# wcaarls/grl

Measured on AMD Instinct MI355X. Metric: env-steps/sec (batched rollouts), pendulum SARSA-tc, higher is better.
Workload: dtype f64

## Files before the change

### grl_amd/csrc/grlx_env_server.h

```cpp
#pragma once

namespace grlx {

struct __attribute__((aligned(16))) MailUnit { double v; unsigned long long seq; };
constexpr int kCandUnits = 5;
constexpr int kCandSlots = 4;
struct __attribute__((aligned(1024))) EnvMail {
  unsigned long long cmd[4];
  MailUnit reset[3];
  unsigned long long pad0[6];
  unsigned long long stats[16];
  union {
    MailUnit by_unit[2][kCandUnits][kCandSlots];
    MailUnit by_cand[2][3][kCandUnits];
  } cand;
  unsigned long long pad1[16];
};
static_assert(sizeof(EnvMail) == kEnvMailBytes, "one mailbox = kEnvMailBytes");
static_assert(offsetof(EnvMail, stats) + 15 * sizeof(unsigned long long) == kEnvMailFlagOffset, "the flag grlx_env_server_counts reads");
static_assert(offsetof(EnvMail, stats) + 14 * sizeof(unsigned long long) == kEnvMailUniformOffset, "the count grlx_uniform_pass_counts reads");

typedef __attribute__((address_space(1))) unsigned long long env_gu64;
typedef unsigned int mail_u32x4 __attribute__((ext_vector_type(4)));
#define GRLX_RLX_AGENT __ATOMIC_RELAXED, __HIP_MEMORY_SCOPE_AGENT
constexpr unsigned kMailReset = 3u, kMailExit = 4u;
constexpr unsigned kFetchPolls = 400u;
constexpr unsigned kFirstFetchPolls = 8000u;
constexpr unsigned kServerStartPolls = 20000u;
constexpr unsigned kServerIdlePolls = 400000u;

__device__ __forceinline__ void mail_store(void *p, unsigned long long v) { __hip_atomic_store((env_gu64 *)p, v, GRLX_RLX_AGENT); }
__device__ __forceinline__ unsigned long long mail_load(const void *p) { return __hip_atomic_load((env_gu64 *)p, GRLX_RLX_AGENT); }
__device__ __forceinline__ void mail_setprio(unsigned p)
{
  if (p == 1) __builtin_amdgcn_s_setprio(1);
  else if (p == 2) __builtin_amdgcn_s_setprio(2);
  else if (p == 3) __builtin_amdgcn_s_setprio(3);
}
__device__ __forceinline__ unsigned long long mail_clock()
{
  unsigned long long t;
  asm volatile("s_memtime %0\n\ts_waitcnt lgkmcnt(0)" : "=s"(t)::"memory");
  return t;
}

__device__ __forceinline__ void unit_store(MailUnit *p, double v, unsigned long long seq)
{
  const unsigned long long b = (unsigned long long)__double_as_longlong(v);
  mail_u32x4 d;
  d.x = (unsigned)b; d.y = (unsigned)(b >> 32); d.z = (unsigned)seq; d.w = (unsigned)(seq >> 32);
  asm volatile("global_store_dwordx4 %0, %1, off sc1\n\ts_nop 1" ::"v"(p), "v"(d) : "memory");
}
template <int I, int STRIDE = 1>
__device__ __forceinline__ void unit_store_at(MailUnit *p, double v, unsigned long long seq)
{
  const unsigned long long b = (unsigned long long)__double_as_longlong(v);
  mail_u32x4 d;
  d.x = (unsigned)b; d.y = (unsigned)(b >> 32); d.z = (unsigned)seq; d.w = (unsigned)(seq >> 32);
  asm volatile("global_store_dwordx4 %0, %1, off offset:%2 sc1\n\ts_nop 1" ::"v"(p), "v"(d), "n"(I * STRIDE * (int)sizeof(MailUnit)) : "memory");
}
template <int N>
__device__ __forceinline__ bool units_load(const MailUnit *p, unsigned long long seq, double *v)
{
  static_assert(N == 3, "");
  mail_u32x4 d[N];
  asm volatile("global_load_dwordx4 %0, %3, off sc1\n\t"
               "global_load_dwordx4 %1, %3, off offset:16 sc1\n\t"
               "global_load_dwordx4 %2, %3, off offset:32 sc1\n\t"
               "s_waitcnt vmcnt(0)"
               : "=&v"(d[0]), "=&v"(d[1]), "=&v"(d[2])
               : "v"(p)
               : "memory");
  bool ok = true;
#pragma unroll
  for (int i = 0; i < N; ++i)
  {
    ok = ok && (((unsigned long long)d[i].w << 32) | d[i].z) == seq;
    v[i] = __longlong_as_double((long long)(((unsigned long long)d[i].y << 32) | d[i].x));
  }
  return ok;
}

struct MailRef {
  EnvMail *all;
  uint32_t r;
  __device__ __forceinline__ EnvMail *get() const { return all + in_reg(r); }
  __device__ __forceinline__ EnvMail *operator->() const { return get(); }
};
__device__ __forceinline__ void mail_send(EnvMail *m, unsigned long long seq, unsigned op) { mail_store(&m->cmd[seq & 3u], (seq << 8) | op); }
__device__ __forceinline__ void mail_send_reset(EnvMail *m, unsigned long long seq, const double *x)
{
  static_assert(offsetof(EnvMail, reset) == 2 * sizeof(MailUnit), "reset[i] is unit 2 + i of the mailbox");
  MailUnit *u = reinterpret_cast<MailUnit *>(m);
  unit_store_at<2>(u, x[0], seq);
  unit_store_at<3>(u, x[1], seq);
  unit_store_at<4>(u, x[2], seq);
  mail_send(m, seq, kMailReset);
}
__device__ __forceinline__ void mail_send(const MailRef &m, unsigned long long seq, unsigned op) { mail_send(m.get(), seq, op); }
__device__ __forceinline__ void mail_send_reset(const MailRef &m, unsigned long long seq, const double *x) { mail_send_reset(m.get(), seq, x); }

template <bool BY_UNIT>
struct MailBox {
  __amdgpu_buffer_rsrc_t rs;
  unsigned at;
};
template <bool BY_UNIT>
__device__ __forceinline__ MailBox<BY_UNIT> mailbox_of(const DevParams &P, int r, int j)
{
  MailBox<BY_UNIT> b;
  b.rs = __builtin_amdgcn_make_buffer_rsrc((void *)P.env_mail, 0, (int)((size_t)P.n_replicas * kEnvMailBytes), 0x00020000);
  b.at = (unsigned)r * (unsigned)kEnvMailBytes + (unsigned)offsetof(EnvMail, cand) + (unsigned)(j < kCandUnits ? j : 0) * (unsigned)((BY_UNIT ? kCandSlots : 1) * sizeof(MailUnit));
  return b;
}
template <bool BY_UNIT>
__device__ __forceinline__ mail_u32x4 mail_prefetch(const MailBox<BY_UNIT> &b, unsigned long long seq, int a)
{
  const unsigned off = BY_UNIT ? b.at + (((unsigned)seq & 1u) * (unsigned)(kCandUnits * kCandSlots) + (unsigned)a) * (unsigned)sizeof(MailUnit)
                               : b.at + (((unsigned)seq & 1u) * 3u + (unsigned)a) * (unsigned)(kCandUnits * sizeof(MailUnit));
  return __builtin_amdgcn_raw_buffer_load_b128(b.rs, off, 0, 16);
}
template <int ENV, bool BY_UNIT>
__device__ __forceinline__ bool mail_take(const DevParams &N, const MailBox<BY_UNIT> &b, mail_u32x4 d, unsigned long long seq, int a, int g,
                                          unsigned long long gmask, double *x, double *obs, double &reward, int &terminal, uint32_t &status,
                                          unsigned long long *polled = nullptr)
{
  static_assert(ENV == GRLX_ENV_PENDULUM, "the pendulum's mailbox");
  bool ok = false;
  unsigned polls = 0;
  for (;;)
  {
    const bool mine = (((unsigned long long)d.w << 32) | d.z) == seq;
    if ((__ballot(mine) & gmask) == gmask) { ok = true; break; }
    if (++polls > (seq <= 1u ? kFirstFetchPolls : kFetchPolls)) break;
    d = mail_prefetch(b, seq, a);
  }
  if (polled) *polled += polls;
  if (!ok) return false;
  const double v = __longlong_as_double((long long)(((unsigned long long)d.y << 32) | d.x));
  const int base = g * 16;
  x[0] = lane_fetch(v, base + 0);
  x[1] = lane_fetch(v, base + 1);
  x[2] = lane_fetch(v, base + 2);
  obs[0] = lane_fetch(v, base + 3);
  obs[1] = x[1];
  reward = lane_fetch(v, base + 4);
  terminal = x[2] > N.timeout ? 1 : 0;
  if (!Env<ENV>::in_domain(x)) status |= ST_DOMAIN;
  return true;
}
template <int ENV, bool BY_UNIT>
__device__ __forceinline__ bool mail_take_wave(const DevParams &N, const MailBox<BY_UNIT> &b, mail_u32x4 d, unsigned long long seq, int a, int g,
                                               double *x, double *obs, double &reward, int &terminal, uint32_t &status,
// ... 24 lines not shown
  return true;
}
__device__ __forceinline__ void mail_nothing_in_flight() { __builtin_amdgcn_s_waitcnt(0x0F70); }
__device__ __forceinline__ mail_u32x4 mail_prefetch_all(const MailBox<true> &b, unsigned long long seq, int j)
{
  const unsigned jj = (j >= kCandUnits && j < 3 * kCandUnits) ? (unsigned)j : 0u;
  const unsigned off = b.at + ((jj % (unsigned)kCandUnits) * (unsigned)kCandSlots + jj / (unsigned)kCandUnits) * (unsigned)sizeof(MailUnit) +
                       ((unsigned)seq & 1u) * (unsigned)(kCandUnits * kCandSlots * sizeof(MailUnit));
  return __builtin_amdgcn_raw_buffer_load_b128(b.rs, off, 0, 16);
}
__device__ __forceinline__ bool mail_vote_all(const MailBox<true> &b, mail_u32x4 &d, unsigned long long seq, int j, unsigned long long *polled = nullptr)
{
  unsigned polls = 0;
  while (!__all((((unsigned long long)d.w << 32) | d.z) == seq))
  {
    if (++polls > kFetchPolls)
    {
      if (polled) *polled += polls;
      return false;
    }
    d = mail_prefetch_all(b, seq, j);
  }
  if (polled) *polled += polls;
  return true;
}
template <int ENV>
__device__ __forceinline__ void mail_hand_round(const DevParams &N, const mail_u32x4 &d, int a, int g, double *x, double *obs, double &reward,
                                                int &terminal, uint32_t &status)
{
  static_assert(ENV == GRLX_ENV_PENDULUM, "the pendulum's mailbox");
  const double v = __longlong_as_double((long long)(((unsigned long long)d.y << 32) | d.x));
  const int base = g * 16 + kCandUnits * a;
  x[0] = lane_fetch(v, base + 0);
  x[1] = lane_fetch(v, base + 1);
  x[2] = lane_fetch(v, base + 2);
  obs[0] = lane_fetch(v, base + 3);
  obs[1] = x[1];
  reward = lane_fetch(v, base + 4);
  terminal = x[2] > N.timeout ? 1 : 0;
  if (!Env<ENV>::in_domain(x)) status |= ST_DOMAIN;
}

template <int ENV, int NA, typename SPEC>
__global__ __launch_bounds__(64) __attribute__((amdgpu_num_vgpr(48))) void env_server_kernel(DevParams P)
{
  static_assert(NA == 3, "sixteen lanes per replica: nine pairs of actions");
  constexpr int S = Env<ENV>::S, D = Env<ENV>::D;
  static_assert(S == 3 && D == 2, "the pendulum's mailbox");
  const DevParams &N = SPEC::numeric(P);
  const int lane = threadIdx.x & 63;
  const int q = lane >> 4, c = lane & 15;
  const int a = c / NA, a2 = c % NA;
  const bool worker = c < NA * NA;
  const int r = blockIdx.x * kReplicasPerWave + q;
  bool done = r >= P.n_replicas || (P.env_tune & 64u) != 0;
  EnvMail *m = P.env_mail + (done ? 0 : r);
  const double act = N.actions[a2];
  unsigned long long expect = 1;
  double cx[S], cobs0 = 0, creward = 0;
#pragma unroll
  for (int i = 0; i < S; ++i) cx[i] = 0;
  unsigned idle = 0;
  bool seen = false;
  mail_setprio((P.env_tune >> 2) & 3u);
  const typename Env<ENV>::ServerConsts ec = Env<ENV>::server_consts();
#ifdef GRLX_ENV_SERVER_STATS
  unsigned long long t_begin = mail_clock(), t_busy = 0, n_cmd = 0, n_idle = 0, n_split = 0, n_batch = 0;
#endif
  const unsigned long long quit_after = (P.env_tune >> 8) & 0xFFFFu;
  const unsigned quit_mask = P.env_tune >> 24;
  const bool leaves = quit_after != 0u && (quit_mask == 0u || ((quit_mask >> q) & 1u) != 0u);
  for (;;)
  {
    if (leaves && expect > quit_after) done = true;
    if (__all(done)) break;
    unsigned long long word = 0;
    bool ready = false;
    if (!done)
    {
      word = mail_load(&m->cmd[expect & 3u]);
      ready = (word >> 8) == expect;
      if ((word >> 8) > expect) done = true;
    }
    if (!__any(ready))
    {
      __builtin_amdgcn_s_sleep(1);
#ifdef GRLX_ENV_SERVER_STATS
      ++n_idle;
#endif
      if (++idle > (seen ? kServerIdlePolls : kServerStartPolls)) break;
      continue;
    }
    seen = true;
    bool progress = false;
#ifdef GRLX_ENV_SERVER_STATS
    const unsigned long long t0 = mail_clock();
    if (!__all(ready || done)) ++n_split;
    ++n_batch;
#endif
    bool step = false;
    unsigned op = 0u;
    if (ready)
    {
      op = (unsigned)(word & 0xFFu);
      if (op == kMailExit)
      {
        done = true;
        progress = true;
      }
      else
        step = true;
    }
    if (rarely(__any(step && op == kMailReset)))
      if (step && op == kMailReset)
      {
        double x[S];
        step = units_load<3>(&m->reset[0], expect, x);
        if (step)
        {
          double obs[D];
          int terminal = 0;
          uint32_t st = 0;
#pragma unroll
          for (int i = 0; i < S; ++i) cx[i] = x[i];
          env_step_consts<ENV>(N, ec, cx, act, obs, creward, terminal, st);
          cobs0 = obs[0];
          op = 0u;
        }
      }
    if (step)
    {
      if (worker && a == (int)op)
      {
        static_assert(NA <= kCandSlots, "slot a2 of every unit is this lane's");
        constexpr bool BY_UNIT = SPEC::kCandByUnit;
        constexpr int STRIDE = BY_UNIT ? kCandSlots : 1;
        MailUnit *u;
        if constexpr (BY_UNIT) u = &m->cand.by_unit[expect & 1u][0][a2];
        else u = &m->cand.by_cand[expect & 1u][a2][0];
        unit_store_at<0, STRIDE>(u, cx[0], expect);
        unit_store_at<1, STRIDE>(u, cx[1], expect);
        unit_store_at<2, STRIDE>(u, cx[2], expect);
        unit_store_at<3, STRIDE>(u, cobs0, expect);
        unit_store_at<4, STRIDE>(u, creward, expect);
      }
      const int src = (lane & ~15) + (int)op * NA + (worker ? a : 0);
      double x[S];
#pragma unroll
      for (int i = 0; i < S; ++i) x[i] = lane_fetch(cx[i], src);
      double obs[D];
      int terminal = 0;
      uint32_t st = 0;
#pragma unroll
      for (int i = 0; i < S; ++i) cx[i] = x[i];
      env_step_consts<ENV>(N, ec, cx, act, obs, creward, terminal, st);
      cobs0 = obs[0];
      ++expect;
      progress = true;
#ifdef GRLX_ENV_SERVER_STATS
      ++n_cmd;
#endif
    }
    if (__any(progress)) idle = 0;
    else if (++idle > kServerIdlePolls) break;
#ifdef GRLX_ENV_SERVER_STATS
    t_busy += mail_clock() - t0;
#endif
  }
#ifdef GRLX_ENV_SERVER_STATS
  if (c == 0 && r < P.n_replicas)
  {
    EnvMail *mm = P.env_mail + r;
    mm->stats[0] = mail_clock() - t_begin;
    mm->stats[1] = t_busy;
    mm->stats[2] = n_cmd;
    mm->stats[3] = n_idle;
    mm->stats[9] = n_split;
    mm->stats[10] = n_batch;
  }
#endif
}

}
```

### grl_amd/csrc/grlx_rollout.h

```cpp
#pragma once

namespace grlx {

__device__ __forceinline__ unsigned long long stamp()
{
  unsigned long long t;
  __builtin_amdgcn_sched_barrier(0);
  asm volatile("s_memtime %0\n\ts_waitcnt lgkmcnt(0)" : "=s"(t)::"memory");
  __builtin_amdgcn_sched_barrier(0);
  return t;
}
#ifdef GRLX_ENV_SERVER_STATS
#define GRLX_STAMPED (DIAG || SERVED)
#else
#define GRLX_STAMPED DIAG
#endif
#define DIAG_STAMP(slot)                                   \
  if (GRLX_STAMPED)                                        \
  {                                                        \
    unsigned long long now__ = stamp();                    \
    diag_sum[slot] += now__ - diag_last;                   \
    diag_last = now__;                                     \
  }

constexpr DevParams make_spec_pendulum_tc()
{
  DevParams P{};
  P.env = GRLX_ENV_PENDULUM;
  P.agent = GRLX_AGENT_SARSA;
  P.trace_kind = GRLX_TRACE_REPLACING;
  P.test_interval = 10;
  P.h = 0.03 / 5;
  P.integration_steps = 5;
  P.timeout = 2.99;
  P.randomization = 0;
  P.A = 3;
  P.actions[0] = -3; P.actions[1] = 0; P.actions[2] = 3;
  P.tile.T = 16; P.tile.D = 3; P.tile.memory = 8388608;
  P.tile.scaling[0] = 16 / 0.31415; P.tile.scaling[1] = 16 / 3.1415; P.tile.scaling[2] = 16 / 3.0;
  P.tile.wrap[0] = 320;
  P.lin.init_min = 0; P.lin.init_range = 1;
  P.lin.out_min = -1.7976931348623157e308; P.lin.out_max = 1.7976931348623157e308;
  P.lin.limit = 1; P.lin.draws_before = 0;
  P.epsilon = 0.05; P.decay_rate = 1; P.decay_min = 0;
  P.alpha = 0.2; P.gamma = 0.97; P.gl = 0.97 * 0.65;
  return P;
}
__device__ const DevParams d_spec_pendulum_tc = make_spec_pendulum_tc();

struct SpecShared {
  static constexpr bool kPerReplica = false;
  static constexpr bool kEarlyTake = false;
  static constexpr bool kCandByUnit = false;
  struct Rep {};
  __device__ static __forceinline__ Rep replica(const SweepParams *, int) { return Rep{}; }
  __device__ static __forceinline__ double alpha(const DevParams &N, const Rep &) { return N.alpha; }
  __device__ static __forceinline__ double gamma(const DevParams &N, const Rep &) { return N.gamma; }
  __device__ static __forceinline__ double gl(const DevParams &N, const Rep &) { return N.gl; }
  __device__ static __forceinline__ double epsilon(const DevParams &N, const Rep &) { return N.epsilon; }
};

template <int AGENT>
struct SpecPendulumTcA : SpecShared {
  static constexpr bool kEarlyTake = true;
  static constexpr bool kCandByUnit = true;
  __device__ static __forceinline__ int agent(const DevParams &) { return AGENT; }
  static bool matches(const DevParams &P)
  {
    constexpr DevParams C = make_spec_pendulum_tc();
    bool ok = P.env == C.env && P.trace_kind == C.trace_kind && P.test_interval == C.test_interval && P.h == C.h &&
              P.integration_steps == C.integration_steps && P.timeout == C.timeout && P.randomization == C.randomization && P.A == C.A &&
              P.tile.T == C.tile.T && P.tile.D == C.tile.D && P.tile.memory == C.tile.memory &&
              P.lin.init_min == C.lin.init_min && P.lin.init_range == C.lin.init_range && P.lin.out_min == C.lin.out_min &&
              P.lin.out_max == C.lin.out_max && P.lin.limit == C.lin.limit && P.lin.draws_before == C.lin.draws_before &&
              P.epsilon == C.epsilon && P.decay_rate == C.decay_rate && P.decay_min == C.decay_min && P.alpha == C.alpha &&
              P.gamma == C.gamma && P.gl == C.gl && P.agent == AGENT;
    for (int i = 0; i < 3; ++i)
      ok = ok && P.actions[i] == C.actions[i] && P.tile.scaling[i] == C.tile.scaling[i] && P.tile.wrap[i] == C.tile.wrap[i];
    return ok;
  }
  __device__ static __forceinline__ const DevParams &numeric(const DevParams &) { return d_spec_pendulum_tc; }
};
using SpecPendulumTc = SpecPendulumTcA<GRLX_AGENT_SARSA>;

inline bool spec_numeric_equal(const DevParams &a, const DevParams &b)
{
  auto tile_eq = [](const TileParams &x, const TileParams &y) {
    bool ok = x.T == y.T && x.D == y.D && x.memory == y.memory;
    for (int i = 0; i < GRLX_MAX_DIMS; ++i) ok = ok && x.scaling[i] == y.scaling[i] && x.wrap[i] == y.wrap[i];
    return ok;
  };
  auto lin_eq = [](const LinearParams &x, const LinearParams &y) {
    return x.init_min == y.init_min && x.init_range == y.init_range && x.out_min == y.out_min && x.out_max == y.out_max &&
           x.limit == y.limit && x.draws_before == y.draws_before;
  };
  bool ok = a.test_interval == b.test_interval && a.env == b.env && a.agent == b.agent && a.trace_kind == b.trace_kind &&
            a.integration_steps == b.integration_steps && a.h == b.h && a.timeout == b.timeout && a.randomization == b.randomization &&
            a.A == b.A && tile_eq(a.tile, b.tile) && lin_eq(a.lin, b.lin) && a.epsilon == b.epsilon && a.decay_rate == b.decay_rate &&
            a.decay_min == b.decay_min && a.alpha == b.alpha && a.gamma == b.gamma && a.gl == b.gl &&
            tile_eq(a.tile_actor, b.tile_actor) && lin_eq(a.lin_actor, b.lin_actor) && a.actor_alpha == b.actor_alpha &&
            a.sigma == b.sigma && a.theta == b.theta && a.ac_decay_rate == b.ac_decay_rate && a.ac_decay_min == b.ac_decay_min &&
            a.ac_step_limit == b.ac_step_limit && a.ac_update_method == b.ac_update_method && a.action_min == b.action_min &&
            a.action_max == b.action_max && a.end_stop_penalty == b.end_stop_penalty && a.action_penalty == b.action_penalty &&
            a.control_step == b.control_step && a.slope_angle == b.slope_angle &&
            a.initial_state_variation == b.initial_state_variation && a.negative_reward == b.negative_reward &&
            a.walker_dt == b.walker_dt && a.kappa == b.kappa && a.beta == b.beta && a.tile_safe == b.tile_safe &&
            a.target_interval == b.target_interval && a.target_tau == b.target_tau;
  for (int i = 0; i < kMaxActions; ++i) ok = ok && a.actions[i] == b.actions[i];
  return ok;
}

constexpr void spec_q_agent_block(DevParams &P)
{
  P.agent = GRLX_AGENT_Q;
  P.trace_kind = GRLX_TRACE_REPLACING;
  P.test_interval = 10;
  P.randomization = 0;
  P.A = 3;
// ... 14 lines not shown
  P.integration_steps = 20;
  P.control_step = 0.2;
  P.h = 0.2 / (double)(size_t)20;
  P.timeout = 100.0;
  P.slope_angle = 0.004; P.initial_state_variation = 0.2; P.negative_reward = -100.0;
  P.walker_dt = 1.0E-6 * (double)(uint64_t)200000 / 20;
  P.action_min = -1.2; P.action_max = 1.2;
  P.actions[0] = -1.2 + (2.4 / 2.) * 0; P.actions[1] = -1.2 + (2.4 / 2.) * 1; P.actions[2] = -1.2 + (2.4 / 2.) * 2;
  P.tile.D = 6;
  P.tile.scaling[0] = 16 / 0.0838; P.tile.scaling[1] = 16 / 0.1047; P.tile.scaling[2] = 16 / 0.1111;
  P.tile.scaling[3] = 16 / 0.2222; P.tile.scaling[4] = 16 / 10.; P.tile.scaling[5] = 16 / 1.2;
  return P;
}
constexpr DevParams make_spec_acrobot_q()
{
  DevParams P{};
  spec_q_agent_block(P);
  P.env = GRLX_ENV_ACROBOT;
  P.integration_steps = 5;
  P.control_step = 0.05;
  P.h = 0.05 / (double)(size_t)5;
  P.timeout = 20.0;
  P.walker_dt = 1.0E-6 * (double)(uint64_t)50000 / 5;
  P.action_min = -1.0; P.action_max = 1.0;
  P.actions[0] = -1.0 + (2.0 / 2.) * 0; P.actions[1] = -1.0 + (2.0 / 2.) * 1; P.actions[2] = -1.0 + (2.0 / 2.) * 2;
  P.tile.D = 5;
  P.tile.scaling[0] = 16 / 0.05; P.tile.scaling[1] = 16 / 0.05; P.tile.scaling[2] = 16 / 0.2; P.tile.scaling[3] = 16 / 0.4;
  P.tile.scaling[4] = 16 / 1.0;
  return P;
}
__device__ const DevParams d_spec_walker_q = make_spec_walker_q();
__device__ const DevParams d_spec_acrobot_q = make_spec_acrobot_q();
struct SpecWalkerQ : SpecShared {
  static constexpr int kEnv = GRLX_ENV_COMPASS_WALKER;
  __device__ static __forceinline__ int agent(const DevParams &) { return GRLX_AGENT_Q; }
  static bool matches(const DevParams &P) { constexpr DevParams C = make_spec_walker_q(); return spec_numeric_equal(P, C); }
  __device__ static __forceinline__ const DevParams &numeric(const DevParams &) { return d_spec_walker_q; }
};
struct SpecAcrobotQ : SpecShared {
  static constexpr int kEnv = GRLX_ENV_ACROBOT;
  __device__ static __forceinline__ int agent(const DevParams &) { return GRLX_AGENT_Q; }
  static bool matches(const DevParams &P) { constexpr DevParams C = make_spec_acrobot_q(); return spec_numeric_equal(P, C); }
  __device__ static __forceinline__ const DevParams &numeric(const DevParams &) { return d_spec_acrobot_q; }
};
struct SpecNone : SpecShared {
  __device__ static __forceinline__ const DevParams &numeric(const DevParams &P) { return P; }
  __device__ static __forceinline__ int agent(const DevParams &P) { return P.agent; }
};
struct SpecSweep {
  __device__ static __forceinline__ const DevParams &numeric(const DevParams &P) { return P; }
  __device__ static __forceinline__ int agent(const DevParams &P) { return P.agent; }
  static constexpr bool kPerReplica = true;
  static constexpr bool kCandByUnit = false;
  struct Rep { double alpha, gamma, gl, epsilon; };
  __device__ static __forceinline__ Rep replica(const SweepParams *sweep, int r)
  {
    const SweepParams &w = sweep[r];
    return Rep{w.alpha, w.gamma, w.gl, w.epsilon};
  }
  __device__ static __forceinline__ double alpha(const DevParams &, const Rep &R) { return R.alpha; }
  __device__ static __forceinline__ double gamma(const DevParams &, const Rep &R) { return R.gamma; }
  __device__ static __forceinline__ double gl(const DevParams &, const Rep &R) { return R.gl; }
  __device__ static __forceinline__ double epsilon(const DevParams &, const Rep &R) { return R.epsilon; }
};

#ifdef GRLX_TWO_WAVES
#define GRLX_ROLLOUT_OCCUPANCY __attribute__((amdgpu_waves_per_eu(2, 2)))
#else
#define GRLX_ROLLOUT_OCCUPANCY
#endif
template <int ENV, int NA, bool DIAG, typename SPEC, bool DEFER, bool ADV, bool TAP, bool SERVED>
__device__ __forceinline__ void rollout_body(const DevParams &P, int n_trials, const SweepParams *sweep = nullptr)
{
  static_assert(!(ADV && DEFER), "the advantage-learning instantiation updates in place");
  constexpr int NROWS = ADV ? 2 * NA : NA + 1;
  const DevParams &N = SPEC::numeric(P);
  constexpr int S = Env<ENV>::S, D = Env<ENV>::D, T = kLanesPerReplica;
  __shared__ double   sh_w[NROWS * 16 * 4];
  __shared__ uint32_t sh_ppos[4 * 16];
  __shared__ double   sh_fb[16 * 4];
  __shared__ uint32_t sh_fbflag[16 * 4];
  __shared__ uint32_t sh_mb[4 * NA * 16];
  __shared__ uint32_t sh_ms[4 * NA * 16];
  __shared__ uint32_t sh_mail[4];
  __shared__ double   sh_res[4 * 16];
  __shared__ uint64_t sh_jump[2048];
  jump_table_to_lds(sh_jump);

  const int lane = threadIdx.x & 63;
  const int g = lane >> 4, j = lane & 15;
  const int r_raw = blockIdx.x * kReplicasPerWave + g;
  const bool live = r_raw < P.n_replicas;
  const int r = live ? r_raw : 0;
  const bool tapped = live && (r == P.tap_replica);
  const unsigned long long gmask = 0xFFFFull << (16 * g);

  ReplicaState &RS = P.states[r];
  double x[S];
#pragma unroll
  for (int i = 0; i < S; ++i) x[i] = RS.x[i];
  uint64_t G = RS.G, TL = RS.TL, S1 = RS.S1;
  double eps_decay = RS.eps_decay;
  int64_t tt = RS.tt, ss = RS.ss;
  uint64_t test_steps = RS.test_steps;
  uint32_t status = RS.status, rows = RS.rows, inserted = 0;

  const typename SPEC::Rep rep = SPEC::replica(sweep, r);
  const Table tab = table_of(P, 0, r);
  ReplicaState RSc;
  RSc.TL0 = RS.TL0;
  RSc.lazy_base[0] = RS.lazy_base[0];
  UpdateParams up;
  up.out_min = N.lin.out_min;
  up.out_max = N.lin.out_max;
  up.limit = N.lin.limit != 0;
  up.ee = SPEC::gl(N, rep);
  up.cut = (N.trace_kind == GRLX_TRACE_REPLACING) ? 0.01 : 0.0001;
  up.use_trace = N.trace_kind == GRLX_TRACE_REPLACING;
  up.dW = up.dT = 0;

  double acts[NA];
#pragma unroll
  for (int a = 0; a < NA; ++a) acts[a] = N.actions[a];
  uint32_t key_act[NA];
#pragma unroll
  for (int a = 0; a < NA; ++a)
    key_act[a] = in_reg(murmur_key(tile_coord<T>(N.tile, D, tile_quant(N.tile, D, N.actions[a]), j)));
  const uint32_t key_j = in_reg(murmur_key(j));

  LaneShare lshare;
  lshare.src[0] = g * 16; lshare.src[1] = g * 16 + 1; lshare.src[2] = g * 16 + 2;
  lshare.role3 = j % 3; lshare.role2 = j & 1;

  constexpr bool EXT = SERVED;
  static_assert(!SERVED || (DEFER && !DIAG && !TAP && !ADV && ENV == GRLX_ENV_PENDULUM && NA == 3), "what the environment server works for");
  MailRef mail = {nullptr, 0u};
  unsigned long long mseq = 0;
  bool srv = false;
  unsigned n_uniform = 0;
#ifdef GRLX_ENV_SERVER_STATS
  unsigned long long st_wait = 0, st_polls = 0, st_fetch = 0, st_begin = mail_clock();
#endif
  MailBox<SPEC::kCandByUnit> mbox;
  mail_u32x4 mpre = {0u, 0u, 0u, 0u};
  if constexpr (EXT)
  {
    srv = live && P.env_mail != nullptr;
    mail = MailRef{P.env_mail, (uint32_t)r};
    mbox = mailbox_of<SPEC::kCandByUnit>(P, r, j);
    mail_setprio(P.env_tune & 3u);
  }

  TraceRegs tr;
  trace_init(tr);
  int tr_len_ref = 0;
  bool pd = false, pd_sh = false;
  double pd_dW = 0, pd_dT = 0, pd_wp = 0;
  uint32_t pd_pos = kInvalidPos;
  unsigned long long diag_sum[8] = {0, 0, 0, 0, 0, 0, 0, 0}, diag_last = 0;
  if (GRLX_STAMPED) diag_last = stamp();

  for (int trial = 0; trial < n_trials; ++trial)
  {
    const bool act = live && !(P.steps_budget != 0u && (uint64_t)ss >= P.steps_budget);
    if (!__any(act)) break;
    const int ti = N.test_interval;
    const int test = (ti >= 0 && tt % (ti + 1) == ti) ? 1 : 0;
    double total_reward = 0, time = 0;
    const int subtrials = (test && P.test_trials > 1) ? P.test_trials : 1;
    for (int st = 0; st < P.test_trials; ++st)
    {
    const bool episode = act && st < subtrials;
    if (!__any(episode)) break;
    double obs[D], reward = 0;
    int terminal = 0;
    bool running = episode;

    if (episode)
    {
      Env<ENV>::start(N, test, TL, G, x);
      Env<ENV>::observe(N, x, obs);
      if constexpr (EXT)
        if (srv)
        {
          ++mseq;
          if (j == 0) mail_send_reset(mail, mseq, x);
        }
    }
    double action = 0;
    int    action_index = 0;
    uint32_t p_pos = kInvalidPos, p_slot = 0;
    bool   p_sh = false;
    double wp_seen = 0;
    uint32_t pos_prev[NA];
#pragma unroll
    for (int a = 0; a < NA; ++a) pos_prev[a] = 0u;
    if (!test) tr_len_ref = 0;
    bool first = true;

    for (;;)
    {
      if constexpr (SERVED)
      {
        static_assert(!Env<ENV>::kAbsorbing, "has_next is taken as true");
        if (__all(live && running && !first && srv && !test && pd) && !(P.env_tune & 16u))
        {
          auto take_classic = [&]() -> bool {
#ifdef GRLX_ENV_SERVER_STATS
            const unsigned long long tf0 = mail_clock();
            const bool stepped = mail_take_wave<ENV>(N, mbox, mpre, mseq - 1, action_index, g, x, obs, reward, terminal, status, &st_polls);
            st_wait += mail_clock() - tf0;
            ++st_fetch;
            return stepped;
#else
            return mail_take_wave<ENV>(N, mbox, mpre, mseq - 1, action_index, g, x, obs, reward, terminal, status);
#endif
          };
          constexpr bool EARLY = SPEC::kEarlyTake;
          bool go = true;
          if constexpr (EARLY)
          {
            DIAG_STAMP(0)
            go = take_classic();
            mail_nothing_in_flight();
          }
          if (go)
          do
          {
            if constexpr (!EARLY)
            {
              DIAG_STAMP(0)
              if (!take_classic()) break;
            }
            ++n_uniform;
            total_reward += reward;
            time += 1;
            DIAG_STAMP(1)

            uint32_t slot[NA];
// ... 117 lines not shown
              }
            }
            auto pass_tail = [&]() {
              DIAG_STAMP(4)
              {
                double target = reward;
                if (SPEC::agent(P) == GRLX_AGENT_SARSA)
                  target += SPEC::gamma(N, rep) * pick<double, NA>(q, a_next);
                else if (SPEC::agent(P) == GRLX_AGENT_EXPECTED_SARSA)
                {
                  const double de = eps_decay * SPEC::epsilon(N, rep);
                  double v = 0;
#pragma unroll
                  for (int kk = 0; kk < NA; ++kk)
                  {
                    double d = (q[kk] == best) ? 1. / man : 0.;
                    if (d == 1) d = 1 - de;
                    d += de / NA;
                    v += q[kk] * d;
                  }
                  target += SPEC::gamma(N, rep) * v;
                }
                else
                {
                  double v = -__builtin_inf();
#pragma unroll
                  for (int kk = 0; kk < NA; ++kk) v = fmax(v, q[kk]);
                  target += SPEC::gamma(N, rep) * v;
                }
                const double delta = target - qsa;
                pd_dW = SPEC::alpha(N, rep) * (target - qsa);
                pd_dT = SPEC::alpha(N, rep) * delta;
                pd_pos = p_pos;
                status |= (p_pos == kInvalidPos) ? ST_BAD_POS : 0u;
                pd_sh = p_sh;
                pd_wp = wp;
              }
              DIAG_STAMP(5)
              ss++;
              action_index = a_next;
              p_pos = pick<uint32_t, NA>(pos, a_next);
              p_sh = pick<bool, NA>(sh, a_next);
              wp_seen = pick<double, NA>(w, a_next);
              if (terminal) running = false;
              if (ev.pos != kInvalidPos) value_store(tab, ev.pos, ev.val);
            };
            if constexpr (EARLY)
            {
              if (!early)
              {
                if (!terminal)
                {
                  ++mseq;
                  if (j == 0) mail_send(mail, mseq, (unsigned)a_next);
                }
                mpre = mail_prefetch(mbox, mseq - 1, a_next);
                DIAG_STAMP(1)
                pass_tail();
                break;
              }
              mail_nothing_in_flight();
              ++mseq;
              if (j == 0) mail_send(mail, mseq, (unsigned)a_next);
              DIAG_STAMP(1)
              pass_tail();
              DIAG_STAMP(0)
              mail_hand_round<ENV>(N, mall, a_next, g, x, obs, reward, terminal, status);
            }
            else
            {
              if (!terminal)
              {
                ++mseq;
                if (j == 0) mail_send(mail, mseq, (unsigned)a_next);
                mpre = mail_prefetch(mbox, mseq - 1, a_next);
              }
              pass_tail();
            }
          } while (EARLY || __all(running));
          action = pick<double, NA>(acts, action_index);
        }
      }
      if (!__any(running || pd)) break;
      uint32_t slot[NA];
      Lookup lk[NA];
      BucketRegs br[NA];
      double wp = 0;
      double wprev[NA];
#pragma unroll
      for (int a = 0; a < NA; ++a) wprev[a] = 0;
      bool has_next = false, update = false;
      if (running)
      {
        DIAG_STAMP(0)
        if (!first)
        {
          bool stepped = false;
          if constexpr (EXT)
            if (srv)
            {
#ifdef GRLX_ENV_SERVER_STATS
              const unsigned long long tf0 = mail_clock();
              stepped = mail_take<ENV>(N, mbox, mpre, mseq - 1, action_index, g, gmask, x, obs, reward, terminal, status, &st_polls);
              st_wait += mail_clock() - tf0;
              ++st_fetch;
#else
              stepped = mail_take<ENV>(N, mbox, mpre, mseq - 1, action_index, g, gmask, x, obs, reward, terminal, status);
#endif
              if (!stepped)
              {
                srv = false;
                ++mseq;
                if (j == 0) mail_send(mail, mseq, kMailExit);
              }
            }
          if (!stepped)
            env_step<ENV, true, LaneShare>(N, x, action, obs, reward, terminal, status, lshare);
          total_reward += reward;
          time += 1;
        }
        has_next = first || !Env<ENV>::kAbsorbing || terminal != 2;
        update = !first && !test;
        DIAG_STAMP(1)

        if (has_next)
        {
          uint32_t hpre = 449u ^ (uint32_t)(D + 2);
#pragma unroll
          for (int i = 0; i < D; ++i)
            hpre = murmur_mix(hpre, tile_coord<T>(N.tile, i, tile_quant(N.tile, i, obs[i]), j));
          const uint32_t hpm = hpre * 0x5bd1e995u;
#pragma unroll
          for (int a = 0; a < NA; ++a)
          {
            uint32_t h = hpm ^ key_act[a];
            h = murmur_absorb(h, key_j);
            const uint32_t hm = murmur_final(h), mem = (uint32_t)N.tile.memory;
            slot[a] = ((mem & (mem - 1u)) == 0u) ? (hm & (mem - 1u)) : (hm % mem);
          }
        }
        DIAG_STAMP(2)
        __builtin_amdgcn_fence(__ATOMIC_SEQ_CST, "workgroup");
        DIAG_STAMP(6)
        if (update) wp = DEFER ? wp_seen : value_load(tab, p_pos);
        if (ADV && update)
        {
#pragma unroll
          for (int a = 0; a < NA; ++a) wprev[a] = value_load(tab, pos_prev[a]);
        }
        if (has_next) table_issue<NA>(tab, slot, lk, br);
      }

      Evicted ev;
      ev.n = 0u; ev.pos = kInvalidPos; ev.val = 0;
      if (DEFER)
      {
        DIAG_STAMP(7)
        if (pd)
        {
          sh_ppos[g * 16 + j] = pd_pos;
          sh_fbflag[j * 4 + g] = 0u;
        }
        wave_sync();
        if (pd)
        {
          up.dW = pd_dW;
// ... 91 lines not shown
          sum /= 16;
          sh_res[g * 16 + j] = sum;
        }
        wave_sync();
        if (has_next)
        {
#pragma unroll
          for (int a = 0; a < NA; ++a) q[a] = clampd(sh_res[g * 16 + a], up.out_min, up.out_max);
        }
        double qsa = 0;
        double qprev[NA];
#pragma unroll
        for (int a = 0; a < NA; ++a) qprev[a] = 0;
        if (update)
        {
          if (ADV)
          {
#pragma unroll
            for (int a = 0; a < NA; ++a) qprev[a] = clampd(sh_res[g * 16 + NA + a], up.out_min, up.out_max);
            qsa = pick<double, NA>(qprev, action_index);
          }
          else
            qsa = clampd(sh_res[g * 16 + NA], up.out_min, up.out_max);
        }

        int a_next = 0;
        int mai = 0, man = 1;
        double best = 0;
        if (has_next)
        {
          findmax<NA>(q, mai, man, best);
          if (test)
          {
            a_next = (man > 1) ? tie_break<NA>(q, best, man, G) : mai;
          }
          else
          {
            if (time == 0.) eps_decay = fmax(eps_decay * N.decay_rate, N.decay_min);
            S1 = lcg_next(S1);
            double rnd = lcg_double(S1);
            if (rnd < eps_decay * SPEC::epsilon(N, rep))
            {
              G = lcg_next(G);
              a_next = (int)(lcg_long(G) % (uint32_t)NA);
            }
            else
              a_next = (man > 1) ? tie_break<NA>(q, best, man, G) : mai;
          }
        }
        if constexpr (EXT)
          if (srv && running && has_next && !(!first && terminal))
          {
            ++mseq;
            if (j == 0) mail_send(mail, mseq, (unsigned)a_next);
            if (!(P.env_tune & 16u))
              mpre = mail_prefetch(mbox, mseq - 1, a_next);
          }

        DIAG_STAMP(4)
        double delta = 0;
        if (update)
        {
          double target = reward;
          if (ADV)
          {
            double v = -__builtin_inf();
#pragma unroll
            for (int kk = 0; kk < NA; ++kk) v = fmax(v, qprev[kk]);
            target = v + (reward - v) / N.kappa;
            if (has_next)
            {
              v = -__builtin_inf();
#pragma unroll
              for (int kk = 0; kk < NA; ++kk) v = fmax(v, q[kk]);
              target += N.gamma * v / N.kappa;
            }
          }
          else if (has_next)
          {
            if (SPEC::agent(P) == GRLX_AGENT_SARSA)
              target += SPEC::gamma(N, rep) * pick<double, NA>(q, a_next);
            else if (SPEC::agent(P) == GRLX_AGENT_EXPECTED_SARSA)
            {
              const double de = eps_decay * SPEC::epsilon(N, rep);
              double v = 0;
#pragma unroll
              for (int kk = 0; kk < NA; ++kk)
              {
                double d = (q[kk] == best) ? 1. / man : 0.;
                if (d == 1) d = 1 - de;
                d += de / NA;
                v += q[kk] * d;
              }
              target += SPEC::gamma(N, rep) * v;
            }
            else
            {
              double v = -__builtin_inf();
#pragma unroll
              for (int kk = 0; kk < NA; ++kk) v = fmax(v, q[kk]);
              target += SPEC::gamma(N, rep) * v;
            }
          }
          delta = target - qsa;
          const double dW = SPEC::alpha(N, rep) * (target - qsa);
          const double dT = SPEC::alpha(N, rep) * delta;
          if (DEFER)
// ... 77 lines not shown
        if (!first && terminal) running = false;
        first = false;
      }
      if (DEFER && ev.pos != kInvalidPos) value_store(tab, ev.pos, ev.val);
    }

    if (!test) trace_flush(tr, tab, true);
    }

    if (act && (ti >= 0 ? test : 1))
    {
      if (rows < (uint32_t)P.max_rows)
      {
        if (j == 0)
        {
          size_t at = (size_t)rows * (size_t)P.n_replicas + (size_t)r;
          P.row_reward[at] = total_reward / (double)subtrials;
          P.row_time[at] = time / (double)subtrials;
          P.row_steps[at] = ss;
          P.row_trial[at] = (ti >= 0) ? (tt + 1 - (tt + 1) / (ti + 1)) : tt;
        }
        rows++;
      }
      else
        status |= ST_ROWS_FULL;
    }
    tt += act ? 1 : 0;
  }

  if (DIAG && P.diag_out && lane == 0)
    for (int k = 0; k < 8; ++k) P.diag_out[(size_t)blockIdx.x * 8 + k] = diag_sum[k];

  if constexpr (EXT)
  {
#ifdef GRLX_ENV_SERVER_STATS
    if (live && j == 0 && P.env_mail)
    {
      mail->stats[4] = mail_clock() - st_begin;
      mail->stats[5] = st_wait;
      mail->stats[6] = st_fetch;
      mail->stats[7] = st_polls;
      mail->stats[8] = srv ? 1 : 0;
      for (int k = 0; k < 8; ++k) mail->pad1[k] = diag_sum[k];
    }
#endif
    if (live && j == 0 && P.env_mail)
    {
      mail->stats[14] = n_uniform;
      mail->stats[15] = srv ? 1u : 2u;
    }
    if (srv)
    {
      ++mseq;
      if (j == 0) mail_send(mail, mseq, kMailExit);
    }
  }

  uint32_t ins = inserted;
#pragma unroll
  for (int off = 8; off > 0; off >>= 1) ins += __shfl_xor(ins, off, 16);
  if (live && j == 0)
  {
#pragma unroll
    for (int i = 0; i < S; ++i) RS.x[i] = x[i];
    RS.G = G;
    RS.TL = TL;
    RS.S1 = S1;
    RS.eps_decay = eps_decay;
    RS.tt = tt;
    RS.ss = ss;
    RS.test_steps = test_steps;
    RS.n_slots[0] += ins;
    RS.rows = rows;
  }
  uint32_t st = status;
#pragma unroll
  for (int off = 8; off > 0; off >>= 1) st |= __shfl_xor(st, off, 16);
  if (live && j == 0) RS.status = st;
}

template <int ENV, int NA, bool DIAG, typename SPEC, bool DEFER = !DIAG, bool ADV = false, bool TAP = !DEFER>
__global__ __launch_bounds__(64) GRLX_ROLLOUT_OCCUPANCY void rollout_kernel(DevParams P, int n_trials)
{
  rollout_body<ENV, NA, DIAG, SPEC, DEFER, ADV, TAP, false>(P, n_trials);
}

template <int ENV, int NA>
__global__ __launch_bounds__(64) GRLX_ROLLOUT_OCCUPANCY void rollout_sweep_kernel(DevParams P, int n_trials, const SweepParams *sweep)
{
  rollout_body<ENV, NA, false, SpecSweep, true, false, false, false>(P, n_trials, sweep);
}

template <int NA, typename SPEC>
__global__ __launch_bounds__(64) __attribute__((amdgpu_num_vgpr(208))) void rollout_served_kernel(DevParams P, int n_trials)
{
  rollout_body<GRLX_ENV_PENDULUM, NA, false, SPEC, true, false, false, true>(P, n_trials);
}


}
```

### grl_amd/runner.py

```python
import collections
import ctypes as C
import math

import numpy as np

from . import capi


def pendulum_sarsa_config(n_replicas=1, **overrides) -> capi.Config:
    lib = capi.load()
    cfg = capi.Config()
    lib.grlx_config_pendulum_sarsa(C.byref(cfg))
    cfg.n_replicas = n_replicas
    for k, v in overrides.items():
        setattr(cfg, k, v)
    return cfg


def cart_pole_ac_config(n_replicas=1, **overrides) -> capi.Config:
    lib = capi.load()
    cfg = capi.Config()
    lib.grlx_config_cart_pole_ac(C.byref(cfg))
    cfg.n_replicas = n_replicas
    for k, v in overrides.items():
# ... 143 lines not shown

    def run_steps(self, max_trials: int, steps: int, stream: int = 0):
        capi.check(self.lib.grlx_run_steps(self._ctx, int(max_trials), int(steps), C.c_void_p(stream)))

    def sync(self, stream: int = 0):
        capi.check(self.lib.grlx_sync(self._ctx, C.c_void_p(stream)))

    def replica_rows(self, replica: int) -> int:
        return capi.check(self.lib.grlx_replica_rows(self._ctx, int(replica)))

    def set_diag(self, enable: bool = True):
        capi.check(self.lib.grlx_set_diag(self._ctx, int(enable)))

    def read_diag(self):
        waves = (self.cfg.n_replicas + 3) // 4
        out = np.zeros((waves, 8), np.uint64)
        n = C.c_int()
        capi.check(self.lib.grlx_read_diag(self._ctx, _ptr(out, C.c_uint64), waves, C.byref(n)))
        return out[: n.value]

    def n_rows(self) -> int:
        return capi.check(self.lib.grlx_rows(self._ctx))

    def rows(self, replica: int, first: int = 0, count: int = None):
        if count is None:
            count = self.replica_rows(replica) - first
        trial = np.zeros(count, np.int64)
        steps = np.zeros(count, np.int64)
        reward = np.zeros(count, np.float64)
        capi.check(self.lib.grlx_read_rows(self._ctx, replica, first, count, _ptr(trial, C.c_int64),
                                           _ptr(steps, C.c_int64), _ptr(reward, C.c_double)))
        return trial, steps, reward

    def last_kernel(self) -> int:
        return self.lib.grlx_last_kernel(self._ctx)

    def last_kernel_name(self) -> str:
        return self.lib.grlx_last_kernel_name(self._ctx).decode()

    def env_server_counts(self):
        a, b = C.c_int(0), C.c_int(0)
        capi.check(self.lib.grlx_env_server_counts(self._ctx, C.byref(a), C.byref(b)))
        return a.value, b.value

    def uniform_pass_counts(self):
        out = np.zeros(self.cfg.n_replicas, dtype=np.uint64)
        capi.check(self.lib.grlx_uniform_pass_counts(self._ctx, _ptr(out, C.c_ulonglong), out.size))
        return out

    def env_server_flags(self):
        out = np.zeros(self.cfg.n_replicas, dtype=np.int32)
        capi.check(self.lib.grlx_env_server_flags(self._ctx, _ptr(out, C.c_int32), out.size))
        return out

    def replicas_per_wave(self) -> int:
        return self.lib.grlx_replicas_per_wave(self._ctx)

    def row_times(self, replica: int, first: int = 0, count: int = None):
        if count is None:
            count = self.n_rows() - first
        out = np.zeros(count, np.float64)
        capi.check(self.lib.grlx_read_row_times(self._ctx, replica, first, count, _ptr(out, C.c_double)))
        return out

    def curve_stats(self, out_dev_ptr: int, first: int, count: int, stream: int = 0):
        capi.check(self.lib.grlx_curve_stats(self._ctx, first, count, C.c_void_p(out_dev_ptr), C.c_void_p(stream)))

    def curve_stats_grouped(self, out_dev_ptr: int, first: int, count: int, group_size: int, stream: int = 0):
        capi.check(self.lib.grlx_curve_stats_grouped(self._ctx, first, count, int(group_size), C.c_void_p(out_dev_ptr), C.c_void_p(stream)))

    def set_replica_params(self, alpha=None, gamma=None, lambda_=None, epsilon=None):
        given = {}
        for name, values in (("alpha", alpha), ("gamma", gamma), ("lambda_", lambda_), ("epsilon", epsilon)):
            if values is None:
                continue
            v = np.ascontiguousarray(values, dtype=np.float64)
            if v.shape != (self.cfg.n_replicas,):
                raise ValueError("need one value per replica")
            given[name] = v
        if not given:
            return
        before = self.replica_params()
        applied = []
        try:
            for name in ("alpha", "epsilon"):
                if name in given:
                    self._set_param(name, given[name])
                    applied.append(name)
            if "gamma" in given and "lambda_" in given:
                applied += ["gamma", "lambda_"]
                self._set_gamma_lambda(before["lambda_"], given["gamma"], given["lambda_"])
            else:
                for name in ("gamma", "lambda_"):
                    if name in given:
                        self._set_param(name, given[name])
        except capi.GrlxError:
            if "gamma" in applied:
                self._set_gamma_lambda(self.replica_params()["lambda_"], before["gamma"], before["lambda_"])
            for name in applied:
                if name in ("alpha", "epsilon"):
                    self._set_param(name, before[name])
            raise

    _PARAMS = {"alpha": capi.PARAM_ALPHA, "gamma": capi.PARAM_GAMMA, "lambda_": capi.PARAM_LAMBDA, "epsilon": capi.PARAM_EPSILON}

    def _set_param(self, name, v):
# ... 528 lines not shown
```

Measured before the change: 781.2 million.

## Pair env-server waves with rollout waves on the same XCC, using local stores

```diff
diff --git a/grl_amd/csrc/grlx_env_server.h b/grl_amd/csrc/grlx_env_server.h
--- a/grl_amd/csrc/grlx_env_server.h
+++ b/grl_amd/csrc/grlx_env_server.h
@@ -59,6 +59,21 @@
   d.x = (unsigned)b; d.y = (unsigned)(b >> 32); d.z = (unsigned)seq; d.w = (unsigned)(seq >> 32);
   asm volatile("global_store_dwordx4 %0, %1, off offset:%2 sc1\n\ts_nop 1" ::"v"(p), "v"(d), "n"(I * STRIDE * (int)sizeof(MailUnit)) : "memory");
 }
+template <int I, int STRIDE = 1>
+__device__ __forceinline__ void unit_store_local_at(MailUnit *p, double v, unsigned long long seq)
+{
+  const unsigned long long b = (unsigned long long)__double_as_longlong(v);
+  mail_u32x4 d;
+  d.x = (unsigned)b; d.y = (unsigned)(b >> 32); d.z = (unsigned)seq; d.w = (unsigned)(seq >> 32);
+  asm volatile("global_store_dwordx4 %0, %1, off offset:%2\n\ts_nop 1" ::"v"(p), "v"(d), "n"(I * STRIDE * (int)sizeof(MailUnit)) : "memory");
+}
+__device__ __forceinline__ void mail_store_local(void *p, unsigned long long v) { __hip_atomic_store((env_gu64 *)p, v, __ATOMIC_RELAXED, __HIP_MEMORY_SCOPE_WAVEFRONT); }
+__device__ __forceinline__ unsigned mail_xcc() { return __builtin_amdgcn_s_getreg(20 | (3 << 11)) & 15u; }
+constexpr int kPairIdWord = 0, kPairClaimWord = 1;
+constexpr unsigned kPairLocalBit = 1u << 24;
+constexpr int kPairGroup = 8;
+enum : unsigned { kPairUnseen = 0u, kPairRemote = 1u, kPairLocal = 2u };
+
 template <int N>
 __device__ __forceinline__ bool units_load(const MailUnit *p, unsigned long long seq, double *v)
 {
@@ -99,6 +114,29 @@
 }
 __device__ __forceinline__ void mail_send(const MailRef &m, unsigned long long seq, unsigned op) { mail_send(m.get(), seq, op); }
 __device__ __forceinline__ void mail_send_reset(const MailRef &m, unsigned long long seq, const double *x) { mail_send_reset(m.get(), seq, x); }
+__device__ __forceinline__ void mail_send(const MailRef &m, unsigned long long seq, unsigned op, unsigned mode)
+{
+  if (mode == kPairLocal) mail_store_local(&m->cmd[seq & 3u], (seq << 8) | op);
+  else mail_send(m.get(), seq, op);
+}
+__device__ __forceinline__ void mail_send_reset(const MailRef &m, unsigned long long seq, const double *x, unsigned mode)
+{
+  if (mode == kPairLocal)
+  {
+    MailUnit *u = reinterpret_cast<MailUnit *>(m.get());
+    unit_store_local_at<2>(u, x[0], seq);
+    unit_store_local_at<3>(u, x[1], seq);
+    unit_store_local_at<4>(u, x[2], seq);
+    mail_store_local(&m->cmd[seq & 3u], (seq << 8) | kMailReset);
+  }
+  else mail_send_reset(m.get(), seq, x);
+}
+__device__ __forceinline__ void mail_publish_xcc(EnvMail *first) { mail_store(&first->pad0[kPairIdWord], (unsigned long long)(mail_xcc() + 1u)); }
+__device__ __forceinline__ unsigned mail_claim_mode(const EnvMail *first)
+{
+  const unsigned w = __builtin_amdgcn_readfirstlane((unsigned)mail_load(&first->pad0[kPairClaimWord]));
+  return w == 0u ? kPairUnseen : (w & kPairLocalBit) ? kPairLocal : kPairRemote;
+}
 
 template <bool BY_UNIT>
 struct MailBox {
@@ -229,7 +267,45 @@
   const int q = lane >> 4, c = lane & 15;
   const int a = c / NA, a2 = c % NA;
   const bool worker = c < NA * NA;
-  const int r = blockIdx.x * kReplicasPerWave + q;
+  unsigned idle = 0;
+  int partner = (int)blockIdx.x;
+  bool local = false;
+  if ((P.env_tune & 64u) == 0u)
+  {
+    const unsigned xcc = mail_xcc();
+    const unsigned base = blockIdx.x & ~(unsigned)(kPairGroup - 1);
+    const unsigned group = min((unsigned)kPairGroup, (unsigned)gridDim.x - base), own = blockIdx.x - base;
+    const bool by_index = (P.env_tune & 128u) != 0u;
+    const bool all_remote = !SPEC::kLocalPair || (P.env_tune & (32u | 128u)) != 0u;
+    unsigned id = (by_index || (unsigned)lane >= group) ? ~0u : 0u;
+    while (!__all(id != 0u))
+    {
+      if (id == 0u) id = (unsigned)mail_load(&P.env_mail[(base + (unsigned)lane) * (unsigned)kReplicasPerWave].pad0[kPairIdWord]);
+      if (__all(id != 0u)) break;
+      __builtin_amdgcn_s_sleep(1);
+      if (++idle > kServerStartPolls) return;
+    }
+    partner = -1;
+    for (unsigned pass = by_index ? 1u : 0u; pass < 2u && partner < 0; ++pass)
+      for (unsigned k = 0; k < (by_index ? 1u : group) && partner < 0; ++k)
+      {
+        const unsigned cand = own + k < group ? own + k : own + k - group;
+        const bool same = (unsigned)__builtin_amdgcn_readlane((int)id, (int)cand) == xcc + 1u;
+        if (pass == 0u && !same) continue;
+        const bool loc = same && !all_remote;
+        unsigned won = 0u;
+        if (lane == 0)
+        {
+          unsigned long long expected = 0ull;
+          const unsigned long long claim = (unsigned long long)(blockIdx.x + 1u) | (loc ? kPairLocalBit : 0u) | ((unsigned long long)(xcc + 1u) << 32);
+          won = __hip_atomic_compare_exchange_strong((env_gu64 *)&P.env_mail[(base + cand) * (unsigned)kReplicasPerWave].pad0[kPairClaimWord], &expected,
+                                                     claim, __ATOMIC_RELAXED, __ATOMIC_RELAXED, __HIP_MEMORY_SCOPE_AGENT) ? 1u : 0u;
+        }
+        if (__builtin_amdgcn_readfirstlane(won) != 0u) { partner = (int)(base + cand); local = loc; }
+      }
+    if (partner < 0) return;
+  }
+  const int r = partner * kReplicasPerWave + q;
   bool done = r >= P.n_replicas || (P.env_tune & 64u) != 0;
   EnvMail *m = P.env_mail + (done ? 0 : r);
   const double act = N.actions[a2];
@@ -237,7 +313,6 @@
   double cx[S], cobs0 = 0, creward = 0;
 #pragma unroll
   for (int i = 0; i < S; ++i) cx[i] = 0;
-  unsigned idle = 0;
   bool seen = false;
   mail_setprio((P.env_tune >> 2) & 3u);
   const typename Env<ENV>::ServerConsts ec = Env<ENV>::server_consts();
@@ -315,11 +390,22 @@
         MailUnit *u;
         if constexpr (BY_UNIT) u = &m->cand.by_unit[expect & 1u][0][a2];
         else u = &m->cand.by_cand[expect & 1u][a2][0];
-        unit_store_at<0, STRIDE>(u, cx[0], expect);
-        unit_store_at<1, STRIDE>(u, cx[1], expect);
-        unit_store_at<2, STRIDE>(u, cx[2], expect);
-        unit_store_at<3, STRIDE>(u, cobs0, expect);
-        unit_store_at<4, STRIDE>(u, creward, expect);
+        if (SPEC::kLocalPair && local)
+        {
+          unit_store_local_at<0, STRIDE>(u, cx[0], expect);
+          unit_store_local_at<1, STRIDE>(u, cx[1], expect);
+          unit_store_local_at<2, STRIDE>(u, cx[2], expect);
+          unit_store_local_at<3, STRIDE>(u, cobs0, expect);
+          unit_store_local_at<4, STRIDE>(u, creward, expect);
+        }
+        else
+        {
+          unit_store_at<0, STRIDE>(u, cx[0], expect);
+          unit_store_at<1, STRIDE>(u, cx[1], expect);
+          unit_store_at<2, STRIDE>(u, cx[2], expect);
+          unit_store_at<3, STRIDE>(u, cobs0, expect);
+          unit_store_at<4, STRIDE>(u, creward, expect);
+        }
       }
       const int src = (lane & ~15) + (int)op * NA + (worker ? a : 0);
       double x[S];
diff --git a/grl_amd/csrc/grlx_rollout.h b/grl_amd/csrc/grlx_rollout.h
--- a/grl_amd/csrc/grlx_rollout.h
+++ b/grl_amd/csrc/grlx_rollout.h
@@ -52,6 +52,7 @@
   static constexpr bool kPerReplica = false;
   static constexpr bool kEarlyTake = false;
   static constexpr bool kCandByUnit = false;
+  static constexpr bool kLocalPair = false;
   struct Rep {};
   __device__ static __forceinline__ Rep replica(const SweepParams *, int) { return Rep{}; }
   __device__ static __forceinline__ double alpha(const DevParams &N, const Rep &) { return N.alpha; }
@@ -64,6 +65,7 @@
 struct SpecPendulumTcA : SpecShared {
   static constexpr bool kEarlyTake = true;
   static constexpr bool kCandByUnit = true;
+  static constexpr bool kLocalPair = true;
   __device__ static __forceinline__ int agent(const DevParams &) { return AGENT; }
   static bool matches(const DevParams &P)
   {
@@ -184,6 +186,7 @@
   __device__ static __forceinline__ int agent(const DevParams &P) { return P.agent; }
   static constexpr bool kPerReplica = true;
   static constexpr bool kCandByUnit = false;
+  static constexpr bool kLocalPair = false;
   struct Rep { double alpha, gamma, gl, epsilon; };
   __device__ static __forceinline__ Rep replica(const SweepParams *sweep, int r)
   {
@@ -269,6 +272,7 @@
   MailRef mail = {nullptr, 0u};
   unsigned long long mseq = 0;
   bool srv = false;
+  unsigned mmode = kPairUnseen;
   unsigned n_uniform = 0;
 #ifdef GRLX_ENV_SERVER_STATS
   unsigned long long st_wait = 0, st_polls = 0, st_fetch = 0, st_begin = mail_clock();
@@ -281,6 +285,7 @@
     mail = MailRef{P.env_mail, (uint32_t)r};
     mbox = mailbox_of<SPEC::kCandByUnit>(P, r, j);
     mail_setprio(P.env_tune & 3u);
+    if (P.env_mail != nullptr && lane == 0) mail_publish_xcc(P.env_mail + blockIdx.x * kReplicasPerWave);
   }
 
   TraceRegs tr;
@@ -308,6 +313,8 @@
     int terminal = 0;
     bool running = episode;
 
+    if constexpr (EXT && SPEC::kLocalPair)
+      if (mmode == kPairUnseen && __any(episode && srv)) mmode = mail_claim_mode(P.env_mail + blockIdx.x * kReplicasPerWave);
     if (episode)
     {
       Env<ENV>::start(N, test, TL, G, x);
@@ -316,7 +323,7 @@
         if (srv)
         {
           ++mseq;
-          if (j == 0) mail_send_reset(mail, mseq, x);
+          if (j == 0) mail_send_reset(mail, mseq, x, mmode);
         }
     }
     double action = 0;
@@ -540,7 +547,7 @@
                 if (!terminal)
                 {
                   ++mseq;
-                  if (j == 0) mail_send(mail, mseq, (unsigned)a_next);
+                  if (j == 0) mail_send(mail, mseq, (unsigned)a_next, mmode);
                 }
                 mpre = mail_prefetch(mbox, mseq - 1, a_next);
                 DIAG_STAMP(1)
@@ -549,7 +556,7 @@
               }
               mail_nothing_in_flight();
               ++mseq;
-              if (j == 0) mail_send(mail, mseq, (unsigned)a_next);
+              if (j == 0) mail_send(mail, mseq, (unsigned)a_next, mmode);
               DIAG_STAMP(1)
               pass_tail();
               DIAG_STAMP(0)
@@ -560,7 +567,7 @@
               if (!terminal)
               {
                 ++mseq;
-                if (j == 0) mail_send(mail, mseq, (unsigned)a_next);
+                if (j == 0) mail_send(mail, mseq, (unsigned)a_next, mmode);
                 mpre = mail_prefetch(mbox, mseq - 1, a_next);
               }
               pass_tail();
@@ -599,7 +606,7 @@
               {
                 srv = false;
                 ++mseq;
-                if (j == 0) mail_send(mail, mseq, kMailExit);
+                if (j == 0) mail_send(mail, mseq, kMailExit, mmode);
               }
             }
           if (!stepped)
@@ -797,7 +804,7 @@
           if (srv && running && has_next && !(!first && terminal))
           {
             ++mseq;
-            if (j == 0) mail_send(mail, mseq, (unsigned)a_next);
+            if (j == 0) mail_send(mail, mseq, (unsigned)a_next, mmode);
             if (!(P.env_tune & 16u))
               mpre = mail_prefetch(mbox, mseq - 1, a_next);
           }
@@ -981,7 +988,7 @@
     if (srv)
     {
       ++mseq;
-      if (j == 0) mail_send(mail, mseq, kMailExit);
+      if (j == 0) mail_send(mail, mseq, kMailExit, mmode);
     }
   }
 
diff --git a/grl_amd/pairing.py b/grl_amd/pairing.py
--- /dev/null
+++ b/grl_amd/pairing.py
@@ -0,0 +1,49 @@
+import numpy as np
+
+MAIL_WORDS = 128
+REPLICAS_PER_WAVE = 4
+GROUP = 8
+ID_WORD, CLAIM_WORD = 10, 11
+PAIR = np.dtype([("claimer", np.int32), ("local", np.bool_), ("rollout_xcc", np.int32), ("server_xcc", np.int32)])
+
+
+def decode_pairing(mail) -> np.ndarray:
+    mail = np.asarray(mail, dtype=np.uint64)
+    if mail.ndim != 2 or mail.shape[1] != MAIL_WORDS:
+        raise ValueError(f"raw mailboxes are uint64 [replicas][{MAIL_WORDS}], not {mail.shape}")
+    first = mail[::REPLICAS_PER_WAVE]
+    ident, claim = first[:, ID_WORD], first[:, CLAIM_WORD]
+    out = np.zeros(first.shape[0], dtype=PAIR)
+    out["claimer"] = (claim & np.uint64(0xFFFFFF)).astype(np.int64) - 1
+    out["local"] = (claim >> np.uint64(24)) & np.uint64(1) != 0
+    out["rollout_xcc"] = (ident & np.uint64(0xFF)).astype(np.int64) - 1
+    out["server_xcc"] = ((claim >> np.uint64(32)) & np.uint64(0xFF)).astype(np.int64) - 1
+    return out
+
+
+def pairing_faults(pairs, by_index=False, all_remote=False) -> list:
+    bad = []
+    n = len(pairs)
+    claimers = [int(c) for c in pairs["claimer"]]
+    for b, c in enumerate(claimers):
+        if c < 0 or c >= n:
+            bad.append(f"block {b}: claimer {c}")
+        elif c // GROUP != b // GROUP:
+            bad.append(f"block {b}: claimer {c} is of another group")
+        if by_index and c != b:
+            bad.append(f"block {b}: claimed by {c} under the pairing by index")
+        if pairs["rollout_xcc"][b] < 0 or (c >= 0 and pairs["server_xcc"][b] < 0):
+            bad.append(f"block {b}: an XCC id is missing")
+        if pairs["local"][b] and pairs["rollout_xcc"][b] != pairs["server_xcc"][b]:
+            bad.append(f"block {b}: local with XCC ids {pairs['rollout_xcc'][b]} and {pairs['server_xcc'][b]}")
+        if pairs["local"][b] and all_remote:
+            bad.append(f"block {b}: local where every claim is remote")
+    if len(set(claimers)) != n:
+        bad.append(f"claimers are not distinct: {claimers}")
+    if not all_remote:
+        for g in range(0, n - GROUP + 1, GROUP):
+            rollout = sorted(int(x) for x in pairs["rollout_xcc"][g:g + GROUP])
+            server = sorted(int(x) for x in pairs["server_xcc"][g:g + GROUP])
+            if len(set(rollout)) == GROUP and rollout == server and not pairs["local"][g:g + GROUP].all():
+                bad.append(f"group {g // GROUP}: one block of each kernel per XCC, but local = {[bool(x) for x in pairs['local'][g:g + GROUP]]}")
+    return bad
diff --git a/grl_amd/runner.py b/grl_amd/runner.py
--- a/grl_amd/runner.py
+++ b/grl_amd/runner.py
@@ -219,6 +219,12 @@
         out = np.zeros(self.cfg.n_replicas, dtype=np.int32)
         capi.check(self.lib.grlx_env_server_flags(self._ctx, _ptr(out, C.c_int32), out.size))
         return out
+
+    def env_server_pairing(self):
+        from .pairing import MAIL_WORDS, decode_pairing
+        mail = np.zeros((self.cfg.n_replicas, MAIL_WORDS), dtype=np.uint64)
+        capi.check(self.lib.grlx_env_server_debug(self._ctx, mail.ctypes.data_as(C.c_void_p), mail.nbytes))
+        return decode_pairing(mail)
 
     def replicas_per_wave(self) -> int:
         return self.lib.grlx_replicas_per_wave(self._ctx)
```

Result: no change. 786.7 million (median of 6 runs) (+0.7%).
